# adeebkor/fenicsx-fus

Hardware: AMD Instinct MI355X
Metric: DOF-updates/sec (RK4 step) at p=4 hex fp64 (higher is better)
Workload: dtype f64; 1 GPU; 3D homogeneous wave, hex p=4 f64, Linear RK4, weak scaling: 64^3 cells per GPU (BASELINE.json configs[1]); ndofs_global=16974593, cells_per_gpu=262144, medium=water, partition=x-slabs x1, transport=none, blocks=8192, mfma_contractions=False, mfma_4x4x4_index1=False, packed_fp32=False, lds_bytes_per_block=72504

## Files before the change

fenicsx-fus_amd/csrc/fusmi.hip:

```cpp
#include <dlfcn.h>

#include <algorithm>
#include <cmath>
#include <cstdio>
#include <cstring>
#include <limits>
#include <memory>

#include "core.hpp"
#include "tables.hpp"

using namespace fus;

FUS_HIDDEN thread_local std::string g_err;
#define NCCLCHK(expr)                                                                              \
  do                                                                                               \
  {                                                                                                \
    ncclResult_t r_ = (expr);                                                                      \
    if (r_ != ncclSuccess)                                                                         \
      return fail(FUS_ERR_RCCL, std::string(#expr) + ": " + g_rccl.GetErrorString(r_));            \
  } while (0)

struct RcclApi
{
// ... 177 lines not shown
  const int Nd = op->Nd, ng = op->tdim == 3 ? 6 : 3;
  FUSCHK(dalloc_bytes(op->allocs, &op->d_G, (size_t)op->ncells * ng * Nd * sizeof(T), false, st));
  FUSCHK(dalloc_bytes(op->allocs, &op->d_detJ, (size_t)op->ncells * Nd * sizeof(T), false, st));
  return degree_impl(op->dtype, op->P)->stream_geometry(op);
}

static OpFacts op_facts(const fus_op* op, int mode, bool ortho, int deterministic)
{
  const fus_ctx* c = op->ctx;
  return {op->P, (int)op->ts, op->tdim, op->geom_order, mode, ortho, deterministic != 0, c->mfma, c->pack32, c->diag_metric};
}

template <typename T>
static int op_setup_device(fus_op* op)
{
  if (!degree_impl(op->dtype, op->P))
    return fail(FUS_ERR_ARG, "unsupported polynomial degree (2..10)");
  const int N = op->N;
  fus_ctx* c = op->ctx;
  hipStream_t st = c->stream;
  Layout& L = op->L;
  auto& pool = op->allocs;

  std::vector<ShapeDev> shapes(L.shapes.size());
  for (size_t i = 0; i < shapes.size(); ++i)
  {
    shapes[i].nelem = L.shapes[i].nelem, shapes[i].nloc = L.shapes[i].nloc;
    shapes[i].nint = L.shapes[i].nint, shapes[i].nrounds = L.shapes[i].nrounds;
    shapes[i].rounds_off = L.shapes[i].rounds_off, shapes[i].ldm_off = L.shapes[i].ldm_off;
  }
  int32_t *d_blk_shape, *d_elem_off, *d_int_off, *d_sh_gidx;
  int64_t* d_sh_off;
  ShapeDev* d_shapes;
  int16_t* d_rounds;
  uint16_t* d_ldm;
  FUSCHK(upload(pool, &d_blk_shape, L.blk_shape, st));
  FUSCHK(upload(pool, &d_shapes, shapes, st));
  FUSCHK(upload(pool, &d_elem_off, L.blk_elem_off, st));
  FUSCHK(upload(pool, &d_int_off, L.blk_int_off, st));
  FUSCHK(upload(pool, &d_sh_off, L.blk_sh_off, st));
  FUSCHK(upload(pool, &d_sh_gidx, L.sh_gidx, st));
  FUSCHK(upload(pool, &d_rounds, L.rounds, st));
  L.ldm.resize((L.ldm.size() + 15) & ~(size_t)15);
  FUSCHK(upload(pool, &d_ldm, L.ldm, st));
  FUSCHK(upload(pool, &op->d_cell_perm, L.cell_perm, st));
  FUSCHK(upload(pool, &op->d_dof_perm, L.dof_perm, st));
  FUSCHK(upload(pool, &op->d_sh_ptr, L.sh_ptr, st));
  {
    std::vector<int64_t> pos(L.sh_pairs.size());
    for (size_t k = 0; k < pos.size(); ++k)
      pos[k] = L.pair_pos[L.sh_pairs[k]];
    FUSCHK(upload(pool, &op->d_sh_pairs, pos, st));
  }
  int32_t* d_sh_ppos;
  FUSCHK(upload(pool, &d_sh_ppos, L.pair_pos, st));
  op->A.sh_ppos = d_sh_ppos;
  op->A.blk_shape = d_blk_shape, op->A.shapes = d_shapes, op->A.blk_elem_off = d_elem_off;
  op->A.blk_int_off = d_int_off, op->A.blk_sh_off = d_sh_off, op->A.sh_gidx = d_sh_gidx;
  op->A.rounds = d_rounds, op->A.ldm = d_ldm, op->A.nblocks = L.nblocks;
  op->A.lds_nloc = (L.max_nloc + 1) & ~1;
  op->A.waves = L.waves;
  op->A.lds_nelem = (L.max_nelem + 7) & ~7;
  op->lds_bytes = L.lds_bytes(sizeof(T), op->nfields);
  if (op->lds_bytes > 160 * 1024)
    return fail(FUS_ERR_LIMIT, "block does not fit 160 KB of LDS; lower block_elems");

  std::vector<T> Dg(N * N + 2 * N);
  for (int i = 0; i < N * N; ++i)
    Dg[i] = (T)op->D[i];
  for (int i = 0; i < N; ++i)
    Dg[N * N + i] = (T)op->wts[i], Dg[N * N + N + i] = (T)op->nodes[i];
  T* d_Dg;
  FUSCHK(upload(pool, &d_Dg, Dg, st));
  op->d_Dg = d_Dg;

  T* d_xg;
  FUSCHK(dalloc(pool, &d_xg, (size_t)op->nnodes * 3));
  HIPCHK(hipMemcpyAsync(d_xg, op->h_geom_x.data(), (size_t)op->nnodes * 3 * sizeof(T),
                        hipMemcpyHostToDevice, st));
  double *d_pts, *d_wts;
  FUSCHK(upload(pool, &op->d_xdm, op->h_geom_dm, st));
// ... 591 lines not shown
    const StageScalars scn = i < 3 ? stage_scalars<T>(m, i + 1, t, dt)
                                   : stage_scalars<T>(m, 0, (double)((T)t + (T)dt), dt);
    B.enabled = 1, B.npairs = (int32_t)op->L.n_partial;
    B.srcw = static_cast<const T*>(m->d_bsrc) + m->nb_int;
    B.absw = static_cast<const T*>(m->d_babs) + m->nb_int;
    B.src2w = m->d_bsrc2 ? static_cast<const T*>(m->d_bsrc2) + m->nb_int : nullptr;
    B.gnext = (T)scn.gval, B.dgnext = (T)scn.dgval;
    B.partial = static_cast<T*>(op->d_partial);
    m->bnd_valid = true, m->bnd_tn = scn.tn;
    op->bnd_owner = m;
    if (m->src_mode == 2)
    {
      B.gnext = T(1), B.dgnext = T(1);
      const bool need_int = !(m->src_tn_int == scn.tn);
      if (need_int || !(m->src_tn_sh == scn.tn))
        FUSCHK(source_entries<T>(m, need_int ? 0 : m->nb_int, m->nb, scn.tn));
    }
  }
  const LeanRK<T> R{(T)sc.b0dt, (T)sc.pdt, T(1) / T(3)};
  const int kind = stage_kind(m, i);
  if (nloc > 0 && c->planes && (int)op->L.plane_cnt.size() <= (c->planes == 1 ? FUS_MAX_PLANES : c->planes))
  {
    ProfScope ps(c, "stage");
    const dim3 grid(nblk(nloc)), blk(256);
    PartialPlanes PL{};
    PL.bnd0 = (int32_t)op->L.n_partial;
    for (size_t j = 0; j < op->L.plane_cnt.size(); ++j)
      PL.cnt[j] = (int32_t)op->L.plane_cnt[j], PL.off[j] = (int32_t)op->L.plane_off[j];
    FUSCHK(with_kind<FUS_STAGE_KINDS>(kind, [&](auto K) -> int
    {
      hipLaunchKernelGGL((k_shared_stage_planes<T, decltype(K)::value>), grid, blk, 0, st, nloc, PL, m->d_bnd_mask, m->d_bnd_base,
                         partial, minv + off, vn + off, un + off, u0 + off, v0 + off, u_ + off, v_ + off, adt, bdt,
                         m0p, mn1p, B, R);
      return FUS_OK;
    }));
  }
  else if (nloc > 0)
  {
    ProfScope ps(c, "stage");
    const dim3 grid(nblk(nloc)), blk(256);
    FUSCHK(with_kind<FUS_STAGE_KINDS>(kind, [&](auto K) -> int
    {
      hipLaunchKernelGGL((k_shared_stage<T, decltype(K)::value>), grid, blk, 0, st, nloc, m->d_sh_ptr32, m->d_sh_pairs32, partial,
                         minv + off, vn + off, un + off, u0 + off, v0 + off, u_ + off, v_ + off, adt, bdt, m0p, mn1p, B,
                         R);
      return FUS_OK;
    }));
// ... 1754 lines not shown
```

fenicsx-fus_amd/csrc/kernels.hpp:

```cpp
#pragma once
#include <hip/hip_runtime.h>
#include <stdint.h>

#include "block_variant.hpp"
#include "geom.hpp"
#include "source_wave.hpp"

namespace fus
{

struct ShapeDev
{
  int32_t nelem, nloc, nint, nrounds;
  int64_t rounds_off, ldm_off;
};

struct BlockArgs
{
  const int32_t* blk_shape;
  const ShapeDev* shapes;
  const int32_t* blk_elem_off;
  const int32_t* blk_int_off;
  const int64_t* blk_sh_off;
  const int32_t* sh_gidx;
  const int32_t* sh_ppos;
  const int16_t* rounds;
  const uint16_t* ldm;
  int32_t nblocks;
  int32_t blk_begin;
  int32_t blk_count;
  int32_t lds_nloc;
  int32_t lds_nelem;
  int32_t waves;
};

template <typename T>
struct StageArgs
{
  const T* minv;
  T *vn, *un, *u0, *v0, *u_, *v_;
  T adt, bdt, gval;
  T b0dt, pdt, third;
  const int32_t* blk_bnd_off;
  const int32_t* bnd_idx;
  const T* bnd_src;
  const T* bnd_abs;
// ... 1854 lines not shown
    for (int j = 0; j < N; ++j)
      acc += Dcc[j] * sA[a * N2 + b * N + j];
    Y[a] = acc;
  }
#pragma unroll
  for (int a = 0; a < N; ++a)
  {
    if (ATOMIC)
      __hip_atomic_fetch_add(&y_l[li[a]], (double)Y[a], __ATOMIC_RELAXED, __HIP_MEMORY_SCOPE_WORKGROUP);
    else
      y_l[li[a]] += Y[a];
  }
}

#define FUS_PF1(T, P, OP, ATOMIC, GEOM, TD)                                                         \
  (((P) >= 5 && (P) <= 7 && (OP) == OP_STIFFNESS && (GEOM) == GEOM_STREAM && (TD) == 3) ? 1 : 0)

template <typename T>
struct LeanRK
{
  T b0dt, pdt, third;
};

template <typename T, int STAGE>
__device__ __forceinline__ T stage_update_dof(int64_t s, T acc, const T* __restrict__ minv,
                                                 T* __restrict__ vn, T* __restrict__ un,
                                                 T* __restrict__ u0, T* __restrict__ v0,
                                                 T* __restrict__ u_, T* __restrict__ v_, T adt, T bdt,
                                                 const T* __restrict__ m0, const T* __restrict__ mn1,
                                                 const LeanRK<T> R)
{
#define FUS_LD(p) __builtin_nontemporal_load(&(p)[s])
#define FUS_ST(p, val) __builtin_nontemporal_store((val), &(p)[s])
  T kv;
  if (mn1)
  {
    const T us = stage_is_first(STAGE) ? u0[s] : un[s], vs = stage_is_first(STAGE) ? v0[s] : vn[s];
    kv = (acc - mn1[s] * vs * vs) / (m0[s] + mn1[s] * us);
  }
  else
    kv = acc * FUS_LD(minv);
  T vnext;
  if (STAGE == 0)
  {
    const T u = FUS_LD(u0), v = FUS_LD(v0);
    FUS_ST(u_, v * bdt + u);
    FUS_ST(v_, kv * bdt + v);
    FUS_ST(un, v * adt + u);
    vnext = kv * adt + v;
    FUS_ST(vn, vnext);
  }
  else if (STAGE == 4)
  {
    const T u = FUS_LD(u0), v = FUS_LD(v0);
    FUS_ST(un, v * adt + u);
    vnext = kv * adt + v;
    FUS_ST(v_, vnext);
  }
  else if (STAGE == 3)
  {
    FUS_ST(u0, FUS_LD(vn) * bdt + FUS_LD(u_));
    vnext = kv * bdt + FUS_LD(v_);
    FUS_ST(v0, vnext);
  }
  else if (STAGE == 5)
  {
    const T w = FUS_LD(vn), v = FUS_LD(v0), xs = FUS_LD(un);
    FUS_ST(un, xs + (w * adt - v * R.pdt));
    vnext = kv * adt + v;
    FUS_ST(v_, vnext);
  }
  else if (STAGE == 6)
  {
    const T w = FUS_LD(vn), v = FUS_LD(v0), va = FUS_LD(u_), xs = FUS_LD(un);
    FUS_ST(un, xs + (w * adt - va * R.pdt));
    vnext = kv * adt + v;
    FUS_ST(v_, vnext);
  }
  else if (STAGE == 7)
  {
    const T w = FUS_LD(vn), v = FUS_LD(v0), va = FUS_LD(u_), vb = FUS_LD(v_), xs = FUS_LD(un);
    FUS_ST(u0, (xs - vb * R.pdt) + ((va + vb) * T(2) + (v + w)) * R.b0dt);
    vnext = kv * bdt + ((vb * T(2) + (va + w)) - v) * R.third;
    FUS_ST(v0, vnext);
  }
  else
  {
    const T w = FUS_LD(vn);
    FUS_ST(u_, w * bdt + FUS_LD(u_));
    FUS_ST(v_, kv * bdt + FUS_LD(v_));
    FUS_ST(un, w * adt + FUS_LD(u0));
    vnext = kv * adt + FUS_LD(v0);
    FUS_ST(vn, vnext);
  }
#undef FUS_LD
#undef FUS_ST
  return vnext;
}

template <typename T, int N>
struct KArgs
{
  BlockArgs A;
  DTab<T, N> Dk;
  const T* Dg;
  const T* geo;
  const T* coef;
  const T* x;
  T* bvec;
  T* partial;
  StageArgs<T> S;
};

template <typename T, int N>
__device__ __forceinline__ void load_stage_args(const KArgs<T, N> __attribute__((address_space(4))) * q, StageArgs<T>& S)
{
  S.minv = q->S.minv;
  S.vn = q->S.vn, S.un = q->S.un, S.u0 = q->S.u0, S.v0 = q->S.v0, S.u_ = q->S.u_, S.v_ = q->S.v_;
  S.adt = q->S.adt, S.bdt = q->S.bdt, S.gval = q->S.gval;
  S.b0dt = q->S.b0dt, S.pdt = q->S.pdt, S.third = q->S.third;
  S.blk_bnd_off = q->S.blk_bnd_off, S.bnd_idx = q->S.bnd_idx;
// ... 49 lines not shown
  uint16_t* ldm_l = reinterpret_cast<uint16_t*>(w_l + (GCS ? (N <= 8 ? 16 : 24) : 0));  \
  int16_t* rt_l = reinterpret_cast<int16_t*>(ldm_l + (size_t)lds_nelem * Nd);                      \
  (void)y_l, (void)x2_l, (void)scratch, (void)D_l, (void)cf_l, (void)cf2_l, (void)gc_l, (void)w_l, (void)pt_l,      \
      (void)ldm_l, (void)rt_l, (void)slots

  const int tid0 = threadIdx.x, nthr = blockDim.x;
#define FUS_TID()                                                                                  \
  int tid = tid0;                                                                                  \
  asm volatile("" : "+v"(tid))
#define FUS_LANE_COORDS(q)                                                                         \
  FUS_TID();                                                                                       \
  const int lane = tid % LPE, wave = tid / LPE;         \
  const int s = lane / N2, p = lane - s * N2;                                                      \
  const int b = p / N, c = p - b * N;                                                              \
  const bool active = s < EPW;                                                                     \
  const int myslot = (wave * EPW + (active ? s : 0)) * EPS;                                        \
                                \
  T* sA = reinterpret_cast<T*>(smem_raw) + (size_t)((NF == 2 ? 2 : 1) + AW) * q->A.lds_nloc         \
          + (size_t)myslot * SLOT;                                                                 \
  T* sB = sA

  struct Meta
  {
    ShapeDev sh;
    int elem_off, int_off;
    int64_t sh_off;
  };
  auto meta_of = [&](KP q, int bk) -> Meta
  {
    Meta M;
    M.sh = q->A.shapes[q->A.blk_shape[bk]];
    M.elem_off = q->A.blk_elem_off[bk];
    M.int_off = q->A.blk_int_off[bk];
    M.sh_off = q->A.blk_sh_off[bk];
    return M;
  };
  typedef T V2 __attribute__((ext_vector_type(2)));
  typedef uint32_t U4 __attribute__((ext_vector_type(4)));
  constexpr int UI = (P <= 3) ? 3 : ((P == 4) ? 2 : (P <= 6 ? 4 : (P == 7 ? FUS_UI_P7 : FUS_UI_HI))),
                US = (P <= 3) ? 4 : ((P == 4) ? 3 : (P <= 7 ? 5 : FUS_UI_HI)),
                UL = (P <= 3) ? 2 : ((P == 4) ? 1 : 4);
  struct PLoad
  {
    V2 xi[UI], xi2[UI];
    T xs[US], xs2[US];
    U4 lq[UL];
    T cfv, cf2v, gcv, gcv2, dgv, xtail, xtail2;
  };
  auto p_idx = [&](KP q, const Meta& M, bool enable, int (&gi)[US]) __attribute__((always_inline))
  {
    FUS_TID();
    const int nsh = M.sh.nloc - M.sh.nint;
    const int32_t* gix = q->A.sh_gidx + M.sh_off;
#pragma unroll
    for (int u = 0; u < US; ++u)
      gi[u] = (enable && tid + u * nthr < nsh) ? gix[tid + u * nthr] : -1;
  };
  auto p_load = [&](KP q, const Meta& M, PLoad& L, bool with_tables, bool enable, const int (&gi)[US])
      __attribute__((always_inline))
  {
    FUS_TID();
    const ShapeDev& sh = M.sh;
    const T* __restrict__ x = q->x;
    const T* __restrict__ x2 = (NF == 2) ? q->S.x2 : x;
    const T* __restrict__ coef = q->coef;
    const T* __restrict__ coef2 = (NF == 2) ? q->S.coef2 : coef;
    const T* __restrict__ geo = q->geo;
    const T* __restrict__ Dg = q->Dg;
    const V2* xg = reinterpret_cast<const V2*>(x + M.int_off);
    const V2* xg2 = reinterpret_cast<const V2*>(x2 + M.int_off);
    const int nvec = sh.nint >> 1;
    const int nsh = sh.nloc - sh.nint;
    const int32_t* gix = q->A.sh_gidx + M.sh_off;
    const int n16 = (sh.nelem * Nd * 2 + 15) >> 4;
    const U4* lsrc = reinterpret_cast<const U4*>(q->A.ldm + sh.ldm_off);
    const int ngc = sh.nelem * GCS;
#pragma unroll
    for (int u = 0; u < UI; ++u)
    {
      const bool ok = enable && tid + u * nthr < nvec;
      L.xi[u] = ok ? xg[tid + u * nthr] : V2(T(0));
      L.xi2[u] = (NF == 2 && ok) ? xg2[tid + u * nthr] : V2(T(0));
    }
#pragma unroll
    for (int u = 0; u < UL; ++u)
      L.lq[u] = (enable && tid + u * nthr < n16) ? lsrc[tid + u * nthr] : U4(0u);
    L.cfv = (enable && tid < sh.nelem) ? coef[M.elem_off + tid] : T(0);
    L.cf2v = (NF == 2 && enable && tid < sh.nelem) ? coef2[M.elem_off + tid] : T(0);
    L.gcv = (enable && tid < ngc) ? geo[(int64_t)M.elem_off * GCS + tid] : T(0);
    L.gcv2 = (GCS > 7 && enable && tid + nthr < ngc) ? geo[(int64_t)M.elem_off * GCS + tid + nthr] : T(0);
    L.dgv = (with_tables && enable && tid < N2 + 2 * N) ? Dg[tid] : T(0);
    L.xtail = (enable && tid == 0 && (sh.nint & 1)) ? x[M.int_off + sh.nint - 1] : T(0);
    L.xtail2 = (NF == 2 && enable && tid == 0 && (sh.nint & 1)) ? x2[M.int_off + sh.nint - 1] : T(0);
#pragma unroll
    for (int u = 0; u < US; ++u)
    {
      L.xs[u] = gi[u] >= 0 ? x[gi[u]] : T(0);
      L.xs2[u] = (NF == 2 && gi[u] >= 0) ? x2[gi[u]] : T(0);
    }
  };
  auto p_commit = [&](KP q, const Meta& M, const PLoad& L, bool with_tables) __attribute__((always_inline))
  {
    FUS_PHASE_LDS(q);
    FUS_TID();
    const ShapeDev& sh = M.sh;
    const T* __restrict__ x = q->x;
    const T* __restrict__ x2 = (NF == 2) ? q->S.x2 : x;
    const T* __restrict__ coef = q->coef;
    const T* __restrict__ coef2 = (NF == 2) ? q->S.coef2 : coef;
    const T* __restrict__ geo = q->geo;
    const T* __restrict__ Dg = q->Dg;
    const V2* xg = reinterpret_cast<const V2*>(x + M.int_off);
    const V2* xg2 = reinterpret_cast<const V2*>(x2 + M.int_off);
    const int nvec = sh.nint >> 1;
    const int nsh = sh.nloc - sh.nint;
    const int32_t* gix = q->A.sh_gidx + M.sh_off;
    const int n16 = (sh.nelem * Nd * 2 + 15) >> 4;
    const U4* lsrc = reinterpret_cast<const U4*>(q->A.ldm + sh.ldm_off);
    const int ngc = sh.nelem * GCS;
    for (int i = tid; i < (sh.nloc + 1) / 2; i += nthr)
      reinterpret_cast<A2*>(y_l)[i] = A2(0.0);
#pragma unroll
    for (int u = 0; u < UI; ++u)
      if (tid + u * nthr < nvec)
      {
        reinterpret_cast<V2*>(x_l)[tid + u * nthr] = L.xi[u];
        if (NF == 2)
          reinterpret_cast<V2*>(x2_l)[tid + u * nthr] = L.xi2[u];
// ... 111 lines not shown
      gc_l[k] = geo[(int64_t)M.elem_off * GCS + k];
    if (!ATOMIC)
      for (int k = tid; k < sh.nrounds * slots; k += nthr)
        rt_l[k] = q->A.rounds[sh.rounds_off + k];
  };

  FUS_KARGS(q0);
  const int blk_end = q0->A.blk_begin + q0->A.blk_count;
  const int blk_stride = gridDim.x;
  int wg = blockIdx.x;
  if (FUS_XCD_REMAP)
  {
    const int G = gridDim.x, q8 = G >> 3, r8 = G & 7, xc = wg & 7;
    wg = xc * q8 + (xc < r8 ? xc : r8) + (wg >> 3);
  }
  int blk = wg + q0->A.blk_begin;
  FUS_STAMP(blk, 0);
  ElemIn<T, N, OP, GEOM, TD> inA, inB;
  auto first_fetch = [&](KP q, const Meta& Mm) __attribute__((always_inline))
  {
    FUS_LANE_COORDS(q);
    (void)b, (void)c, (void)sA, (void)sB;
    const int slots = (q->A.waves * 64 / LPE) * EPW * EPS;
    const int nt0 = ATOMIC ? (Mm.sh.nelem + slots - 1) / slots : Mm.sh.nrounds;
    int e0 = -1;
    if (active && nt0 > 0)
      e0 = ATOMIC ? (myslot < Mm.sh.nelem ? myslot : -1) : (int)q->A.rounds[Mm.sh.rounds_off + myslot];
    elem_fetch<T, N, OP, GEOM, TD>(inA, e0, q->geo, Mm.elem_off, p);
  };
  PLoad L;
  {
    const Meta M0 = meta_of(q0, blk);
    first_fetch(q0, M0);
    int gi0[US];
    p_idx(q0, M0, true, gi0);
    p_load(q0, M0, L, true, true, gi0);
  }
  bool first = true;
  for (;;)
  {
  FUS_KARGS(qc);
  FUS_PHASE_LDS(qc);
  FUS_LANE_COORDS(qc);
  const Meta M = meta_of(qc, blk);
  const ShapeDev& sh = M.sh;
  const int elem_off = M.elem_off;
  const int ntrips = ATOMIC ? (sh.nelem + slots - 1) / slots : sh.nrounds;
  auto elem_of = [&](int r) -> int
  {
    if (!active || r >= ntrips)
      return -1;
    if (ATOMIC)
      return (r * slots + myslot < sh.nelem) ? r * slots + myslot : -1;
    return (int)rt_l[r * slots + myslot];
  };
#ifdef FUS_PROBE_PFREE
  if (first)
    p_commit(qc, M, L, true);
  else
  {
    FUS_TID();
    for (int i = tid; i < (M.sh.nloc + 1) / 2; i += nthr)
      reinterpret_cast<A2*>(y_l)[i] = A2(0.0);
  }
#else
  p_commit(qc, M, L, first);
#endif
  const int blk_next = blk + blk_stride;
  const bool has_next = blk_next < blk_end;
  constexpr bool IDX_EARLY = false;
  int gi_n[US];
  if constexpr (IDX_EARLY)
  {
    Meta Mi{};
    if (has_next)
      Mi = meta_of(qc, blk_next);
    p_idx(qc, Mi, has_next, gi_n);
  }
  __syncthreads();
  FUS_STAMP(blk, 1);
#ifdef FUS_STAGGER
  if (tid0 >= 256)
    __builtin_amdgcn_s_sleep(FUS_STAGGER);
#endif
  T Drb[N], Drc[N], Dcb[N], Dcc[N], w3[N];
// ... 83 lines not shown
    FUS_ELEM_COMPUTE(inA);
    if (r == 0)
      FUS_STAMP(blk, 5);
    if (r == 2)
      FUS_STAMP(blk, 7);
    if (!ATOMIC && nwaves > 1)
      __syncthreads();
    elem_fetch<T, N, OP, GEOM, TD>(inA, elem_of(r + 2), geo, elem_off, p);
    if (has1)
    {
      FUS_ELEM_COMPUTE(inB);
      if (r == 0)
        FUS_STAMP(blk, 6);
      if (!ATOMIC && nwaves > 1)
        __syncthreads();
    }
  }
#undef FUS_ELEM_COMPUTE
  {
  FUS_KARGS(qe);
  FUS_PHASE_LDS(qe);
  FUS_TID();
  const Meta M = meta_of(qe, blk);
  const ShapeDev& sh = M.sh;
  const int int_off = M.int_off;
  const int64_t sh_off = M.sh_off;
  StageArgs<T> S;
  load_stage_args<T, N>(qe, S);
  T* __restrict__ bvec = qe->bvec;
  T* __restrict__ partial = qe->partial;
  const int32_t* __restrict__ pp = qe->A.sh_ppos + sh_off;
  const int nsh = sh.nloc - sh.nint;
  int ppv[US];
#pragma unroll
  for (int u = 0; u < US; ++u)
    ppv[u] = (tid + u * nthr < nsh) ? pp[tid + u * nthr] : -1;

  const int nvec = sh.nint >> 1;
    constexpr bool EPI2 = (P <= 4) && (NF == 1);
    struct Epi
    {
      bool on;
      int i, o;
      V2 bv, mi, w, a0, b0, au, av, m1, m0v, us;
    };
    auto epi_load = [&](int i, Epi& E, int part) __attribute__((always_inline))
    {
      if (part != 2)
      {
      E.on = i < nvec;
      E.i = i, E.o = int_off + 2 * i;
      E.bv = E.mi = E.w = E.a0 = E.b0 = E.au = E.av = E.m1 = E.m0v = E.us = V2(T(0));
#ifdef FUS_PROBE_EFREE
      auto ld = [&](const T* ptr) -> V2 { return E.on ? V2(T(1)) + V2(T((uintptr_t)ptr & 7)) : V2(T(0)); };
#else
      auto ld = [&](const T* ptr) -> V2
      { return E.on ? __builtin_nontemporal_load(reinterpret_cast<const V2*>(ptr + E.o)) : V2(T(0)); };
#endif
      constexpr bool WV = NF == 2;
// ... 100 lines not shown
#ifdef FUS_PROBE_PFREE
    if constexpr (!IDX_EARLY)
      p_idx(qn, Mn, false, gi_n);
    p_load(qn, Mn, L, false, false, gi_n);
#else
    if constexpr (!IDX_EARLY)
      p_idx(qn, Mn, has_next, gi_n);
    p_load(qn, Mn, L, false, has_next, gi_n);
#endif
  }
  if (STAGE == STAGE_NONE)
  {
    V2* bg = reinterpret_cast<V2*>(bvec + int_off);
    for (int i = tid; i < nvec; i += nthr)
    {
      const A2 a2 = reinterpret_cast<const A2*>(y_l)[i];
      bg[i] = V2{(T)a2[0], (T)a2[1]};
    }
    if (tid == 0 && (sh.nint & 1))
      bvec[int_off + sh.nint - 1] = (T)y_l[sh.nint - 1];
  }
  else
  {
    const int k0 = S.blk_bnd_off[blk], k1 = S.blk_bnd_off[blk + 1];
    if (k1 > k0)
    {
      const T* vstage = stage_is_first(STAGE) ? S.v0 : S.vn;
      for (int k = k0 + tid; k < k1; k += nthr)
      {
        const int gi = S.bnd_idx[k];
        T add = S.gval * S.bnd_src[k] - S.bnd_abs[k] * vstage[gi];
        if (NF == 2)
          add += S.dgval * S.bnd_src2[k];
        y_l[gi - int_off] += add;
      }
      __syncthreads();
    }
    if (tid == 0 && (sh.nint & 1))
      (void)stage_update_dof<T, STAGE>((int64_t)int_off + sh.nint - 1, (T)y_l[sh.nint - 1], S.minv, S.vn, S.un, S.u0,
                                       S.v0, S.u_, S.v_, S.adt, S.bdt, (NF == 2) ? S.m0 : nullptr,
                                       (NF == 2) ? S.mn1 : nullptr, LeanRK<T>{S.b0dt, S.pdt, S.third});
#pragma unroll
    for (int u = 0; u < EPIU; ++u)
      epi_load(tid + u * nthr, Ef[u], EARLY ? 2 : 0);
#pragma unroll
    for (int u = 0; u < EPIU; ++u)
      epi_store(Ef[u]);
// ... 41 lines not shown
{
  const int64_t s = s0 + (int64_t)blockIdx.x * blockDim.x + threadIdx.x;
  if (s >= s1)
    return;
  T acc = T(0);
  for (I k = sh_ptr[s]; k < sh_ptr[s + 1]; ++k)
    acc += partial[sh_pairs[k]];
  bsh[s] = acc;
}

template <typename T>
struct BndNext
{
  int enabled;
  int32_t npairs;
  const T *srcw, *absw, *src2w;
  T gnext, dgnext;
  T* partial;
};

template <typename T>
__device__ __forceinline__ void boundary_next(const BndNext<T>& B, int32_t last_pair, T vnext)
{
  if (B.enabled && last_pair >= B.npairs)
  {
    const int32_t k = last_pair - B.npairs;
    T v = B.gnext * B.srcw[k] - B.absw[k] * vnext;
    if (B.src2w)
      v += B.dgnext * B.src2w[k];
    B.partial[last_pair] = v;
  }
}



constexpr int FUS_MAX_PLANES = 16;
struct PartialPlanes
{
  int32_t bnd0;
  int32_t cnt[FUS_MAX_PLANES];
  int32_t off[FUS_MAX_PLANES];
};

template <typename T, int STAGE>
__global__ void __launch_bounds__(256)
k_shared_stage_planes(int64_t n, const PartialPlanes PL, const uint64_t* __restrict__ bnd_mask,
                      const int32_t* __restrict__ bnd_base, const T* __restrict__ partial,
                      const T* __restrict__ minv, T* __restrict__ vn, T* __restrict__ un, T* __restrict__ u0,
                      T* __restrict__ v0, T* __restrict__ u_, T* __restrict__ v_, T adt, T bdt,
                      const T* __restrict__ m0, const T* __restrict__ mn1, const BndNext<T> B, const LeanRK<T> R)
{
  const int64_t s = (int64_t)blockIdx.x * blockDim.x + threadIdx.x;
  if (s >= n)
    return;
  T acc = T(0);
#pragma unroll
  for (int j = 0; j < FUS_MAX_PLANES; ++j)
  {
    if (s < PL.cnt[j])
      acc += partial[(int64_t)PL.off[j] + s];
  }
  int32_t pair = -1;
  if (bnd_mask)
  {
    const uint64_t w = bnd_mask[s >> 6];
    const int bit = (int)(s & 63);
    if ((w >> bit) & 1ull)
    {
      pair = PL.bnd0 + bnd_base[s >> 6] + __builtin_popcountll(w & ((1ull << bit) - 1ull));
      acc += partial[pair];
    }
  }
  const T vnext = stage_update_dof<T, STAGE>(s, acc, minv, vn, un, u0, v0, u_, v_, adt, bdt, m0, mn1, R);
  boundary_next<T>(B, pair, vnext);
}

template <typename T, int STAGE>
__global__ void __launch_bounds__(256)
k_shared_stage(int64_t n, const int32_t* __restrict__ sh_ptr, const int32_t* __restrict__ sh_pairs,
               const T* __restrict__ partial, const T* __restrict__ minv, T* __restrict__ vn,
               T* __restrict__ un, T* __restrict__ u0, T* __restrict__ v0, T* __restrict__ u_,
               T* __restrict__ v_, T adt, T bdt, const T* __restrict__ m0,
               const T* __restrict__ mn1, const BndNext<T> B, const LeanRK<T> R)
{
  const int64_t s = (int64_t)blockIdx.x * blockDim.x + threadIdx.x;
  if (s >= n)
    return;
  T acc = T(0);
  int32_t pair = 0;
  for (int32_t k = sh_ptr[s]; k < sh_ptr[s + 1]; ++k)
  {
    pair = sh_pairs[k];
    acc += partial[pair];
  }
  const T vnext = stage_update_dof<T, STAGE>(s, acc, minv, vn, un, u0, v0, u_, v_, adt, bdt, m0, mn1, R);
  boundary_next<T>(B, pair, vnext);
}
// ... 428 lines not shown
```

fenicsx-fus_amd/csrc/layout.cpp:

```cpp
#include "layout.hpp"

#include <algorithm>
#include <cstring>
#include <map>
#include <numeric>
#include <unordered_map>

namespace fus
{
namespace
{
struct Rcb
{
  const double* cen;
  std::vector<int32_t>& order;
  std::vector<std::pair<int64_t, int64_t>>& leaves;

  void split(int64_t lo, int64_t hi, int64_t nparts)
  {
    if (nparts <= 1 || hi - lo <= 1)
    {
      leaves.emplace_back(lo, hi);
      return;
    }
// ... 328 lines not shown
        const int64_t mid = (lo + hi) / 2;
        if (L.sh_ptr[mid + 1] - L.sh_ptr[mid] > j)
          lo = mid + 1;
        else
          hi = mid;
      }
      cnt = lo;
    }
    if (cnt == 0)
      break;
    L.plane_cnt.push_back(cnt), L.plane_off.push_back(cursor);
    cursor = (cursor + cnt + 15) & ~(int64_t)15;
  }
  L.pair_pos.assign(L.npairs, -1);
  for (int64_t sidx = 0; sidx < L.n_shared_local; ++sidx)
    for (int64_t k = L.sh_ptr[sidx]; k < L.sh_ptr[sidx + 1]; ++k)
      L.pair_pos[L.sh_pairs[k]] = (int32_t)(L.plane_off[k - L.sh_ptr[sidx]] + sidx);
  const int64_t if_first = L.sh_ptr[std::min(L.n_if_start_pad, L.n_shared)];
  for (int64_t k = if_first; k < L.npairs; ++k)
    L.pair_pos[L.sh_pairs[k]] = (int32_t)(cursor + (k - if_first));
  L.n_partial = cursor + (L.npairs - if_first);
  if (L.n_partial + L.n_shared > 2000000000ll)
    return "partial slab exceeds int32 indexing";
  return "";
}

std::string verify_layout(const Layout& L, const int32_t* dm)
{
  const int Nd = L.Nd;
  {
    std::vector<uint8_t> seen(L.ncells, 0);
    for (int64_t e = 0; e < L.ncells; ++e)
    {
      const int32_t c = L.cell_perm[e];
      if (c < 0 || c >= L.ncells || seen[c])
        return "cell_perm is not a permutation";
      seen[c] = 1;
    }
  }
  {
    std::vector<uint8_t> seen(L.n_internal, 0);
    for (int64_t g = 0; g < L.ndofs; ++g)
    {
      const int32_t p = L.dof_perm[g];
      if (p < 0 || p >= L.n_internal || seen[p])
        return "dof_perm is not injective";
      seen[p] = 1;
// ... 34 lines not shown
        if (e >= sh.nelem || used[e]++)
          return "round table does not cover each element once";
        for (int i = 0; i < Nd; ++i)
          if (stamp[L.ldm[sh.ldm_off + (int64_t)e * Nd + i]] == r)
            return "two elements of one round share a dof";
        for (int i = 0; i < Nd; ++i)
          stamp[L.ldm[sh.ldm_off + (int64_t)e * Nd + i]] = r;
      }
    for (int e = 0; e < sh.nelem; ++e)
      if (!used[e])
        return "element missing from rounds";
    pairs_seen += sh.nloc - sh.nint;
  }
  if (pairs_seen != L.npairs)
    return "pair count mismatch";
  {
    std::vector<char> taken(L.n_partial, 0);
    for (int64_t k = 0; k < L.npairs; ++k)
    {
      if (L.pair_pos[k] < 0 || L.pair_pos[k] >= L.n_partial || taken[L.pair_pos[k]]++)
        return "two pairs share a partial position";
    }
  }
  for (int64_t s = 0; s < L.n_shared; ++s)
    for (int64_t k = L.sh_ptr[s]; k < L.sh_ptr[s + 1]; ++k)
    {
      if (L.sh_gidx[L.sh_pairs[k]] != L.n_int_pad + s)
        return "shared CSR inconsistent";
      if (k > L.sh_ptr[s] && L.sh_pairs[k] <= L.sh_pairs[k - 1])
        return "shared CSR not in ascending block order";
      const int64_t pos = L.pair_pos[L.sh_pairs[k]], j = k - L.sh_ptr[s];
      if (pos < 0 || pos >= L.n_partial)
        return "partial position out of range";
      if (s < L.n_shared_local && (j >= (int64_t)L.plane_cnt.size() || s >= L.plane_cnt[j] || pos != L.plane_off[j] + s))
        return "partial position is not (plane of the sharer's rank, dof index)";
    }
  return "";
}

}
```

fenicsx-fus_amd/csrc/layout.hpp:

```cpp
#pragma once
#include <cstdint>
#include <string>
#include <vector>

namespace fus
{

struct Layout
{
  int P = 0, N = 0, Nd = 0;
  int tdim = 3;
  int waves = 4;
  int epw = 1;
  int slots = 4;
  int64_t ncells = 0, ndofs = 0;

  int32_t nblocks = 0;
  int32_t nblocks_if = 0;
  std::vector<int32_t> cell_perm;
  std::vector<int32_t> blk_elem_off;

  struct Shape
  {
    int32_t nelem, nloc, nint, nrounds;
    int64_t rounds_off;
    int64_t ldm_off;
  };
  std::vector<Shape> shapes;
  std::vector<int32_t> blk_shape;
  std::vector<int16_t> rounds;
  std::vector<uint16_t> ldm;

  std::vector<int32_t> dof_perm;
  std::vector<int32_t> blk_int_off;
  std::vector<int64_t> blk_sh_off;
  std::vector<int32_t> sh_gidx;
  int64_t n_int_pad = 0;
  int64_t n_interior = 0, n_shared = 0, npairs = 0;
  int64_t n_shared_local = 0, n_if_start_pad = 0;
  int64_t n_internal = 0;
  std::vector<int64_t> sh_ptr;
  std::vector<int64_t> sh_pairs;
  std::vector<int32_t> pair_pos;
  std::vector<int64_t> plane_cnt, plane_off;
  int64_t n_partial = 0;
  int32_t max_nloc = 0, max_rounds = 0, max_nelem = 0;

  size_t lds_bytes(size_t sizeofT, int nfields = 1, int geom_cell_stride = 0) const
  {
    const size_t ne = ((size_t)max_nelem + 7) & ~(size_t)7;
    return (size_t)nfields * ((max_nloc + 1) & ~1) * sizeofT
           + (size_t)((max_nloc + 1) & ~1) * 8
           + (size_t)slots * ((tdim == 3 && N == 7 && sizeofT == 4) ? N * 56 : Nd + N) * sizeofT
           + (size_t)N * N * sizeofT + nfields * ne * sizeofT
           + (geom_cell_stride ? ((size_t)geom_cell_stride * ne + (N <= 8 ? 16 : 24)) * sizeofT : 0)
           + ne * Nd * 2
           + (size_t)max_rounds * slots * 2 + 16;
  }
};

std::string build_layout(Layout& L, int P, int64_t ncells, int64_t ndofs,
                         const int32_t* tensor_dofmap, const double* centroids, int block_elems,
                         int waves, const uint8_t* force_shared = nullptr, int tdim = 3, int slot_factor = 1);

std::string verify_layout(const Layout& L, const int32_t* tensor_dofmap);

}
```

Baseline: 13.71 billion DOF-updates/s.

## Vectorize shared-DOF stage update and pack per-block metadata into cache-line records

The shared/plane stage kernel now handles several DOFs per thread (16-byte vectors) and uses vector nontemporal loads and stores for partial planes and the RK state arrays, with scalar fallbacks for tails. Per-block metadata that used to be gathered from five separate arrays is packed into one 64-byte BlockRecord and read through the constant address space. The boundary offsets are also loaded early, and the RK update arithmetic is rewritten with explicit FMAs under fp contract(off). In return the code adds a plane-alignment requirement and changes rounding slightly because of the explicit FMAs.

```diff
diff --git a/fenicsx-fus_amd/csrc/fusmi.hip b/fenicsx-fus_amd/csrc/fusmi.hip
--- a/fenicsx-fus_amd/csrc/fusmi.hip
+++ b/fenicsx-fus_amd/csrc/fusmi.hip
@@ -223,23 +223,11 @@
   Layout& L = op->L;
   auto& pool = op->allocs;
 
-  std::vector<ShapeDev> shapes(L.shapes.size());
-  for (size_t i = 0; i < shapes.size(); ++i)
-  {
-    shapes[i].nelem = L.shapes[i].nelem, shapes[i].nloc = L.shapes[i].nloc;
-    shapes[i].nint = L.shapes[i].nint, shapes[i].nrounds = L.shapes[i].nrounds;
-    shapes[i].rounds_off = L.shapes[i].rounds_off, shapes[i].ldm_off = L.shapes[i].ldm_off;
-  }
-  int32_t *d_blk_shape, *d_elem_off, *d_int_off, *d_sh_gidx;
-  int64_t* d_sh_off;
-  ShapeDev* d_shapes;
+  int32_t* d_sh_gidx;
+  BlockRecord* d_blk_rec;
   int16_t* d_rounds;
   uint16_t* d_ldm;
-  FUSCHK(upload(pool, &d_blk_shape, L.blk_shape, st));
-  FUSCHK(upload(pool, &d_shapes, shapes, st));
-  FUSCHK(upload(pool, &d_elem_off, L.blk_elem_off, st));
-  FUSCHK(upload(pool, &d_int_off, L.blk_int_off, st));
-  FUSCHK(upload(pool, &d_sh_off, L.blk_sh_off, st));
+  FUSCHK(upload(pool, &d_blk_rec, L.blk_rec, st));
   FUSCHK(upload(pool, &d_sh_gidx, L.sh_gidx, st));
   FUSCHK(upload(pool, &d_rounds, L.rounds, st));
   L.ldm.resize((L.ldm.size() + 15) & ~(size_t)15);
@@ -256,8 +244,7 @@
   int32_t* d_sh_ppos;
   FUSCHK(upload(pool, &d_sh_ppos, L.pair_pos, st));
   op->A.sh_ppos = d_sh_ppos;
-  op->A.blk_shape = d_blk_shape, op->A.shapes = d_shapes, op->A.blk_elem_off = d_elem_off;
-  op->A.blk_int_off = d_int_off, op->A.blk_sh_off = d_sh_off, op->A.sh_gidx = d_sh_gidx;
+  op->A.blk_rec = d_blk_rec, op->A.sh_gidx = d_sh_gidx;
   op->A.rounds = d_rounds, op->A.ldm = d_ldm, op->A.nblocks = L.nblocks;
   op->A.lds_nloc = (L.max_nloc + 1) & ~1;
   op->A.waves = L.waves;
@@ -895,7 +882,8 @@
   if (nloc > 0 && c->planes && (int)op->L.plane_cnt.size() <= (c->planes == 1 ? FUS_MAX_PLANES : c->planes))
   {
     ProfScope ps(c, "stage");
-    const dim3 grid(nblk(nloc)), blk(256);
+    constexpr int W = 16 / (int)sizeof(T);
+    const dim3 grid(nblk((nloc + W - 1) / W)), blk(256);
     PartialPlanes PL{};
     PL.bnd0 = (int32_t)op->L.n_partial;
     for (size_t j = 0; j < op->L.plane_cnt.size(); ++j)
diff --git a/fenicsx-fus_amd/csrc/kernels.hpp b/fenicsx-fus_amd/csrc/kernels.hpp
--- a/fenicsx-fus_amd/csrc/kernels.hpp
+++ b/fenicsx-fus_amd/csrc/kernels.hpp
@@ -4,24 +4,15 @@
 
 #include "block_variant.hpp"
 #include "geom.hpp"
+#include "layout.hpp"
 #include "source_wave.hpp"
 
 namespace fus
 {
 
-struct ShapeDev
-{
-  int32_t nelem, nloc, nint, nrounds;
-  int64_t rounds_off, ldm_off;
-};
-
 struct BlockArgs
 {
-  const int32_t* blk_shape;
-  const ShapeDev* shapes;
-  const int32_t* blk_elem_off;
-  const int32_t* blk_int_off;
-  const int64_t* blk_sh_off;
+  const BlockRecord* blk_rec;
   const int32_t* sh_gidx;
   const int32_t* sh_ppos;
   const int16_t* rounds;
@@ -1922,81 +1913,181 @@
   T b0dt, pdt, third;
 };
 
+enum : int { SR_MINV = 1, SR_M0 = 2, SR_MN1 = 4, SR_U0 = 8, SR_V0 = 16, SR_UN = 32, SR_VN = 64, SR_UA = 128, SR_VA = 256 };
+__host__ __device__ constexpr int stage_reads(int st, bool wv)
+{
+  return ((st == 0 || st == 4) ? SR_U0 | SR_V0
+          : st == 3            ? SR_VN | SR_UA | SR_VA
+          : st == 5            ? SR_VN | SR_V0 | SR_UN
+          : st == 6            ? SR_VN | SR_V0 | SR_UA | SR_UN
+          : st == 7            ? SR_VN | SR_V0 | SR_UA | SR_VA | SR_UN
+                               : SR_VN | SR_UA | SR_VA | SR_U0 | SR_V0)
+         | (wv ? SR_M0 | SR_MN1 | (stage_is_first(st) ? SR_U0 | SR_V0 : SR_UN | SR_VN) : SR_MINV);
+}
+__host__ __device__ constexpr int stage_writes(int st)
+{
+  return (st == 3 || st == 7) ? SR_U0 | SR_V0 : (st >= 4 ? SR_UN | SR_VA : SR_UA | SR_VA | SR_UN | SR_VN);
+}
+
+template <typename T>
+struct StageRegs
+{
+  T minv, m0, mn1, u0, v0, un, vn, ua, va;
+};
+
+__device__ __forceinline__ double fmadd(double a, double b, double c) { return __builtin_fma(a, b, c); }
+__device__ __forceinline__ float fmadd(float a, float b, float c) { return __builtin_fmaf(a, b, c); }
+
+__host__ __device__ constexpr int stage_kv_reads(int st, bool wv)
+{
+  return wv ? SR_M0 | SR_MN1 | (stage_is_first(st) ? SR_U0 | SR_V0 : SR_UN | SR_VN) : SR_MINV;
+}
 template <typename T, int STAGE>
-__device__ __forceinline__ T stage_update_dof(int64_t s, T acc, const T* __restrict__ minv,
+__device__ __forceinline__ T stage_kv(T acc, bool wv, const StageRegs<T>& r)
+{
+#pragma clang fp contract(off)
+  if (wv)
+  {
+    const T us = stage_is_first(STAGE) ? r.u0 : r.un, vs = stage_is_first(STAGE) ? r.v0 : r.vn;
+    return fmadd(-vs, r.mn1 * vs, acc) / fmadd(r.mn1, us, r.m0);
+  }
+  return acc * r.minv;
+}
+template <typename T, int STAGE>
+__device__ __forceinline__ T stage_finish(T kv, StageRegs<T>& r, T adt, T bdt, const LeanRK<T> R)
+{
+#pragma clang fp contract(off)
+  T vnext;
+  if (STAGE == 0)
+  {
+    const T u = r.u0, v = r.v0;
+    r.ua = fmadd(v, bdt, u);
+    r.va = fmadd(kv, bdt, v);
+    r.un = fmadd(v, adt, u);
+    vnext = fmadd(kv, adt, v);
+    r.vn = vnext;
+  }
+  else if (STAGE == 4)
+  {
+    const T u = r.u0, v = r.v0;
+    r.un = fmadd(v, adt, u);
+    vnext = fmadd(kv, adt, v);
+    r.va = vnext;
+  }
+  else if (STAGE == 3)
+  {
+    r.u0 = fmadd(r.vn, bdt, r.ua);
+    vnext = fmadd(kv, bdt, r.va);
+    r.v0 = vnext;
+  }
+  else if (STAGE == 5)
+  {
+    const T w = r.vn, v = r.v0, xs = r.un;
+    r.un = xs + fmadd(w, adt, -(v * R.pdt));
+    vnext = fmadd(kv, adt, v);
+    r.va = vnext;
+  }
+  else if (STAGE == 6)
+  {
+    const T w = r.vn, v = r.v0, va = r.ua, xs = r.un;
+    r.un = xs + fmadd(w, adt, -(va * R.pdt));
+    vnext = fmadd(kv, adt, v);
+    r.va = vnext;
+  }
+  else if (STAGE == 7)
+  {
+    const T w = r.vn, v = r.v0, va = r.ua, vb = r.va, xs = r.un;
+    r.u0 = fmadd(fmadd(va + vb, T(2), v + w), R.b0dt, fmadd(-vb, R.pdt, xs));
+    vnext = fmadd(kv, bdt, (fmadd(vb, T(2), va + w) - v) * R.third);
+    r.v0 = vnext;
+  }
+  else
+  {
+    const T w = r.vn, ua = r.ua, va = r.va;
+    r.ua = fmadd(w, bdt, ua);
+    r.va = fmadd(kv, bdt, va);
+    r.un = fmadd(w, adt, r.u0);
+    vnext = fmadd(kv, adt, r.v0);
+    r.vn = vnext;
+  }
+  return vnext;
+}
+template <typename T, int STAGE>
+__device__ __forceinline__ T stage_update_regs(T acc, bool wv, StageRegs<T>& r, T adt, T bdt, const LeanRK<T> R)
+{
+  return stage_finish<T, STAGE>(stage_kv<T, STAGE>(acc, wv, r), r, adt, bdt, R);
+}
+
+#define FUS_STAGE_VECTORS(X)                                                                        \
+  X(minv, minv, SR_MINV) X(m0, m0, SR_M0) X(mn1, mn1, SR_MN1) X(u0, u0, SR_U0) X(v0, v0, SR_V0)     \
+  X(un, un, SR_UN) X(vn, vn, SR_VN) X(ua, u_, SR_UA) X(va, v_, SR_VA)
+template <typename T, int STAGE, typename V = T>
+__device__ __forceinline__ V stage_update_dof(int64_t s, V acc, const T* __restrict__ minv,
                                                  T* __restrict__ vn, T* __restrict__ un,
                                                  T* __restrict__ u0, T* __restrict__ v0,
                                                  T* __restrict__ u_, T* __restrict__ v_, T adt, T bdt,
                                                  const T* __restrict__ m0, const T* __restrict__ mn1,
-                                                 const LeanRK<T> R)
-{
-#define FUS_LD(p) __builtin_nontemporal_load(&(p)[s])
-#define FUS_ST(p, val) __builtin_nontemporal_store((val), &(p)[s])
-  T kv;
-  if (mn1)
-  {
-    const T us = stage_is_first(STAGE) ? u0[s] : un[s], vs = stage_is_first(STAGE) ? v0[s] : vn[s];
-    kv = (acc - mn1[s] * vs * vs) / (m0[s] + mn1[s] * us);
+                                                 const LeanRK<T> R, int nv = (int)(sizeof(V) / sizeof(T)))
+{
+  constexpr int W = (int)(sizeof(V) / sizeof(T));
+  const bool wv = mn1 != nullptr;
+  const bool whole = W == 1 || nv == W;
+  StageRegs<V> q{};
+  const int reads = stage_reads(STAGE, wv);
+  auto load = [&](int mask) __attribute__((always_inline))
+  {
+#define FUS_LD(f, p, bit)                                                                           \
+  if (reads & mask & (bit))                                                                         \
+  {                                                                                                 \
+    if (whole)                                                                                      \
+      q.f = __builtin_nontemporal_load(reinterpret_cast<const V*>(&(p)[s]));                        \
+    else if constexpr (W > 1)                                                                       \
+      for (int e = 0; e < W; ++e)                                                                   \
+        if (e < nv)                                                                                 \
+          q.f[e] = __builtin_nontemporal_load(&(p)[s + e]);                                         \
+  }
+    FUS_STAGE_VECTORS(FUS_LD)
+#undef FUS_LD
+  };
+  V vnext;
+  if constexpr (W == 1)
+  {
+    load(stage_kv_reads(STAGE, wv));
+    const T kv = stage_kv<T, STAGE>(acc, wv, q);
+    load(~stage_kv_reads(STAGE, wv));
+    vnext = stage_finish<T, STAGE>(kv, q, adt, bdt, R);
   }
   else
-    kv = acc * FUS_LD(minv);
-  T vnext;
-  if (STAGE == 0)
-  {
-    const T u = FUS_LD(u0), v = FUS_LD(v0);
-    FUS_ST(u_, v * bdt + u);
-    FUS_ST(v_, kv * bdt + v);
-    FUS_ST(un, v * adt + u);
-    vnext = kv * adt + v;
-    FUS_ST(vn, vnext);
-  }
-  else if (STAGE == 4)
-  {
-    const T u = FUS_LD(u0), v = FUS_LD(v0);
-    FUS_ST(un, v * adt + u);
-    vnext = kv * adt + v;
-    FUS_ST(v_, vnext);
-  }
-  else if (STAGE == 3)
-  {
-    FUS_ST(u0, FUS_LD(vn) * bdt + FUS_LD(u_));
-    vnext = kv * bdt + FUS_LD(v_);
-    FUS_ST(v0, vnext);
-  }
-  else if (STAGE == 5)
-  {
-    const T w = FUS_LD(vn), v = FUS_LD(v0), xs = FUS_LD(un);
-    FUS_ST(un, xs + (w * adt - v * R.pdt));
-    vnext = kv * adt + v;
-    FUS_ST(v_, vnext);
-  }
-  else if (STAGE == 6)
-  {
-    const T w = FUS_LD(vn), v = FUS_LD(v0), va = FUS_LD(u_), xs = FUS_LD(un);
-    FUS_ST(un, xs + (w * adt - va * R.pdt));
-    vnext = kv * adt + v;
-    FUS_ST(v_, vnext);
-  }
-  else if (STAGE == 7)
-  {
-    const T w = FUS_LD(vn), v = FUS_LD(v0), va = FUS_LD(u_), vb = FUS_LD(v_), xs = FUS_LD(un);
-    FUS_ST(u0, (xs - vb * R.pdt) + ((va + vb) * T(2) + (v + w)) * R.b0dt);
-    vnext = kv * bdt + ((vb * T(2) + (va + w)) - v) * R.third;
-    FUS_ST(v0, vnext);
-  }
-  else
-  {
-    const T w = FUS_LD(vn);
-    FUS_ST(u_, w * bdt + FUS_LD(u_));
-    FUS_ST(v_, kv * bdt + FUS_LD(v_));
-    FUS_ST(un, w * adt + FUS_LD(u0));
-    vnext = kv * adt + FUS_LD(v0);
-    FUS_ST(vn, vnext);
-  }
-#undef FUS_LD
+  {
+    load(~0);
+#pragma unroll
+    for (int e = 0; e < W; ++e)
+    {
+      StageRegs<T> r;
+#define FUS_GET(f, p, bit) r.f = q.f[e];
+      FUS_STAGE_VECTORS(FUS_GET)
+#undef FUS_GET
+      vnext[e] = stage_update_regs<T, STAGE>(acc[e], wv, r, adt, bdt, R);
+#define FUS_PUT(f, p, bit) q.f[e] = r.f;
+      FUS_STAGE_VECTORS(FUS_PUT)
+#undef FUS_PUT
+    }
+  }
+#define FUS_ST(f, p, bit)                                                                           \
+  if constexpr ((stage_writes(STAGE) & (bit)) != 0)                                                 \
+  {                                                                                                 \
+    if (whole)                                                                                      \
+      __builtin_nontemporal_store(q.f, reinterpret_cast<V*>(const_cast<T*>(&(p)[s])));              \
+    else if constexpr (W > 1)                                                                       \
+      for (int e = 0; e < W; ++e)                                                                   \
+        if (e < nv)                                                                                 \
+          __builtin_nontemporal_store(q.f[e], const_cast<T*>(&(p)[s + e]));                         \
+  }
+  FUS_STAGE_VECTORS(FUS_ST)
 #undef FUS_ST
   return vnext;
 }
+#undef FUS_STAGE_VECTORS
 
 template <typename T, int N>
 struct KArgs
@@ -2092,17 +2183,19 @@
 
   struct Meta
   {
-    ShapeDev sh;
-    int elem_off, int_off;
+    int32_t elem_off, int_off;
     int64_t sh_off;
+    int32_t nelem, nloc, nint, nrounds;
+    int64_t rounds_off, ldm_off;
   };
   auto meta_of = [&](KP q, int bk) -> Meta
   {
+    const BlockRecord __attribute__((address_space(4)))* r
+        = (const BlockRecord __attribute__((address_space(4)))*)q->A.blk_rec + bk;
     Meta M;
-    M.sh = q->A.shapes[q->A.blk_shape[bk]];
-    M.elem_off = q->A.blk_elem_off[bk];
-    M.int_off = q->A.blk_int_off[bk];
-    M.sh_off = q->A.blk_sh_off[bk];
+    M.elem_off = r->elem_off, M.int_off = r->int_off, M.sh_off = r->sh_off;
+    M.nelem = r->nelem, M.nloc = r->nloc, M.nint = r->nint, M.nrounds = r->nrounds;
+    M.rounds_off = r->rounds_off, M.ldm_off = r->ldm_off;
     return M;
   };
   typedef T V2 __attribute__((ext_vector_type(2)));
@@ -2120,7 +2213,7 @@
   auto p_idx = [&](KP q, const Meta& M, bool enable, int (&gi)[US]) __attribute__((always_inline))
   {
     FUS_TID();
-    const int nsh = M.sh.nloc - M.sh.nint;
+    const int nsh = M.nloc - M.nint;
     const int32_t* gix = q->A.sh_gidx + M.sh_off;
 #pragma unroll
     for (int u = 0; u < US; ++u)
@@ -2130,7 +2223,7 @@
       __attribute__((always_inline))
   {
     FUS_TID();
-    const ShapeDev& sh = M.sh;
+    const Meta& sh = M;
     const T* __restrict__ x = q->x;
     const T* __restrict__ x2 = (NF == 2) ? q->S.x2 : x;
     const T* __restrict__ coef = q->coef;
@@ -2173,7 +2266,7 @@
   {
     FUS_PHASE_LDS(q);
     FUS_TID();
-    const ShapeDev& sh = M.sh;
+    const Meta& sh = M;
     const T* __restrict__ x = q->x;
     const T* __restrict__ x2 = (NF == 2) ? q->S.x2 : x;
     const T* __restrict__ coef = q->coef;
@@ -2331,10 +2424,10 @@
     FUS_LANE_COORDS(q);
     (void)b, (void)c, (void)sA, (void)sB;
     const int slots = (q->A.waves * 64 / LPE) * EPW * EPS;
-    const int nt0 = ATOMIC ? (Mm.sh.nelem + slots - 1) / slots : Mm.sh.nrounds;
+    const int nt0 = ATOMIC ? (Mm.nelem + slots - 1) / slots : Mm.nrounds;
     int e0 = -1;
     if (active && nt0 > 0)
-      e0 = ATOMIC ? (myslot < Mm.sh.nelem ? myslot : -1) : (int)q->A.rounds[Mm.sh.rounds_off + myslot];
+      e0 = ATOMIC ? (myslot < Mm.nelem ? myslot : -1) : (int)q->A.rounds[Mm.rounds_off + myslot];
     elem_fetch<T, N, OP, GEOM, TD>(inA, e0, q->geo, Mm.elem_off, p);
   };
   PLoad L;
@@ -2352,7 +2445,7 @@
   FUS_PHASE_LDS(qc);
   FUS_LANE_COORDS(qc);
   const Meta M = meta_of(qc, blk);
-  const ShapeDev& sh = M.sh;
+  const Meta& sh = M;
   const int elem_off = M.elem_off;
   const int ntrips = ATOMIC ? (sh.nelem + slots - 1) / slots : sh.nrounds;
   auto elem_of = [&](int r) -> int
@@ -2369,7 +2462,7 @@
   else
   {
     FUS_TID();
-    for (int i = tid; i < (M.sh.nloc + 1) / 2; i += nthr)
+    for (int i = tid; i < (M.nloc + 1) / 2; i += nthr)
       reinterpret_cast<A2*>(y_l)[i] = A2(0.0);
   }
 #else
@@ -2499,7 +2592,7 @@
   FUS_PHASE_LDS(qe);
   FUS_TID();
   const Meta M = meta_of(qe, blk);
-  const ShapeDev& sh = M.sh;
+  const Meta& sh = M;
   const int int_off = M.int_off;
   const int64_t sh_off = M.sh_off;
   StageArgs<T> S;
@@ -2512,6 +2605,12 @@
 #pragma unroll
   for (int u = 0; u < US; ++u)
     ppv[u] = (tid + u * nthr < nsh) ? pp[tid + u * nthr] : -1;
+  int bnd_k0 = 0, bnd_k1 = 0;
+  if (STAGE != STAGE_NONE)
+  {
+    const int32_t __attribute__((address_space(4)))* bo = (const int32_t __attribute__((address_space(4)))*)S.blk_bnd_off + blk;
+    bnd_k0 = bo[0], bnd_k1 = bo[1];
+  }
 
   const int nvec = sh.nint >> 1;
     constexpr bool EPI2 = (P <= 4) && (NF == 1);
@@ -2658,7 +2757,12 @@
   }
   else
   {
+#ifdef FUS_PROBE_BND_LATE
     const int k0 = S.blk_bnd_off[blk], k1 = S.blk_bnd_off[blk + 1];
+    (void)bnd_k0, (void)bnd_k1;
+#else
+    const int k0 = bnd_k0, k1 = bnd_k1;
+#endif
     if (k1 > k0)
     {
       const T* vstage = stage_is_first(STAGE) ? S.v0 : S.vn;
@@ -2746,12 +2850,13 @@
 template <typename T>
 __device__ __forceinline__ void boundary_next(const BndNext<T>& B, int32_t last_pair, T vnext)
 {
+#pragma clang fp contract(off)
   if (B.enabled && last_pair >= B.npairs)
   {
     const int32_t k = last_pair - B.npairs;
-    T v = B.gnext * B.srcw[k] - B.absw[k] * vnext;
+    T v = fmadd(B.gnext, B.srcw[k], -(B.absw[k] * vnext));
     if (B.src2w)
-      v += B.dgnext * B.src2w[k];
+      v = fmadd(B.dgnext, B.src2w[k], v);
     B.partial[last_pair] = v;
   }
 }
@@ -2774,29 +2879,64 @@
                       T* __restrict__ v0, T* __restrict__ u_, T* __restrict__ v_, T adt, T bdt,
                       const T* __restrict__ m0, const T* __restrict__ mn1, const BndNext<T> B, const LeanRK<T> R)
 {
-  const int64_t s = (int64_t)blockIdx.x * blockDim.x + threadIdx.x;
+  constexpr int W = 16 / (int)sizeof(T);
+  typedef T V __attribute__((ext_vector_type(W)));
+  const int64_t s = ((int64_t)blockIdx.x * blockDim.x + threadIdx.x) * W;
   if (s >= n)
     return;
-  T acc = T(0);
+  T acc[W];
+#pragma unroll
+  for (int e = 0; e < W; ++e)
+    acc[e] = T(0);
 #pragma unroll
   for (int j = 0; j < FUS_MAX_PLANES; ++j)
   {
-    if (s < PL.cnt[j])
-      acc += partial[(int64_t)PL.off[j] + s];
-  }
-  int32_t pair = -1;
+    const int64_t cnt = PL.cnt[j], off = PL.off[j];
+    if (s + W <= cnt)
+    {
+      const V v = __builtin_nontemporal_load(reinterpret_cast<const V*>(partial + off + s));
+#pragma unroll
+      for (int e = 0; e < W; ++e)
+        acc[e] += v[e];
+    }
+    else
+    {
+#pragma unroll
+      for (int e = 0; e < W; ++e)
+        if (s + e < cnt)
+          acc[e] += partial[off + s + e];
+    }
+  }
+  int32_t pair[W];
+#pragma unroll
+  for (int e = 0; e < W; ++e)
+    pair[e] = -1;
   if (bnd_mask)
   {
     const uint64_t w = bnd_mask[s >> 6];
-    const int bit = (int)(s & 63);
-    if ((w >> bit) & 1ull)
-    {
-      pair = PL.bnd0 + bnd_base[s >> 6] + __builtin_popcountll(w & ((1ull << bit) - 1ull));
-      acc += partial[pair];
-    }
-  }
-  const T vnext = stage_update_dof<T, STAGE>(s, acc, minv, vn, un, u0, v0, u_, v_, adt, bdt, m0, mn1, R);
-  boundary_next<T>(B, pair, vnext);
+    const int bit0 = (int)(s & 63);
+    if ((w >> bit0) & ((1ull << W) - 1ull))
+    {
+      const int32_t base = PL.bnd0 + bnd_base[s >> 6];
+#pragma unroll
+      for (int e = 0; e < W; ++e)
+        if ((w >> (bit0 + e)) & 1ull)
+        {
+          pair[e] = base + __builtin_popcountll(w & ((1ull << (bit0 + e)) - 1ull));
+          acc[e] += partial[pair[e]];
+        }
+    }
+  }
+  V av;
+#pragma unroll
+  for (int e = 0; e < W; ++e)
+    av[e] = acc[e];
+  const int nv = (n - s < W) ? (int)(n - s) : W;
+  const V vnext = stage_update_dof<T, STAGE, V>(s, av, minv, vn, un, u0, v0, u_, v_, adt, bdt, m0, mn1, R, nv);
+#pragma unroll
+  for (int e = 0; e < W; ++e)
+    if (e < nv)
+      boundary_next<T>(B, pair[e], vnext[e]);
 }
 
 template <typename T, int STAGE>
diff --git a/fenicsx-fus_amd/csrc/layout.cpp b/fenicsx-fus_amd/csrc/layout.cpp
--- a/fenicsx-fus_amd/csrc/layout.cpp
+++ b/fenicsx-fus_amd/csrc/layout.cpp
@@ -374,7 +374,22 @@
   L.n_partial = cursor + (L.npairs - if_first);
   if (L.n_partial + L.n_shared > 2000000000ll)
     return "partial slab exceeds int32 indexing";
+  L.blk_rec = block_records(L);
   return "";
+}
+
+std::vector<BlockRecord> block_records(const Layout& L)
+{
+  std::vector<BlockRecord> rec(L.nblocks);
+  for (int32_t b = 0; b < L.nblocks; ++b)
+  {
+    const Layout::Shape& sh = L.shapes[L.blk_shape[b]];
+    BlockRecord& r = rec[b];
+    r.elem_off = L.blk_elem_off[b], r.int_off = L.blk_int_off[b], r.sh_off = L.blk_sh_off[b];
+    r.nelem = sh.nelem, r.nloc = sh.nloc, r.nint = sh.nint, r.nrounds = sh.nrounds;
+    r.rounds_off = sh.rounds_off, r.ldm_off = sh.ldm_off;
+  }
+  return rec;
 }
 
 std::string verify_layout(const Layout& L, const int32_t* dm)
@@ -455,6 +470,11 @@
         return "two pairs share a partial position";
     }
   }
+  for (int64_t off : L.plane_off)
+    if (off % 16)
+      return "plane not aligned";
+  if ((int64_t)L.blk_rec.size() != L.nblocks)
+    return "block records missing";
   for (int64_t s = 0; s < L.n_shared; ++s)
     for (int64_t k = L.sh_ptr[s]; k < L.sh_ptr[s + 1]; ++k)
     {
diff --git a/fenicsx-fus_amd/csrc/layout.hpp b/fenicsx-fus_amd/csrc/layout.hpp
--- a/fenicsx-fus_amd/csrc/layout.hpp
+++ b/fenicsx-fus_amd/csrc/layout.hpp
@@ -5,6 +5,16 @@
 
 namespace fus
 {
+
+struct alignas(64) BlockRecord
+{
+  int32_t elem_off, int_off;
+  int64_t sh_off;
+  int32_t nelem, nloc, nint, nrounds;
+  int64_t rounds_off, ldm_off;
+  uint8_t pad[16] = {};
+};
+static_assert(sizeof(BlockRecord) == 64 && alignof(BlockRecord) == 64, "one cache line per block");
 
 struct Layout
 {
@@ -28,6 +38,7 @@
   };
   std::vector<Shape> shapes;
   std::vector<int32_t> blk_shape;
+  std::vector<BlockRecord> blk_rec;
   std::vector<int16_t> rounds;
   std::vector<uint16_t> ldm;
 
@@ -63,6 +74,8 @@
                          const int32_t* tensor_dofmap, const double* centroids, int block_elems,
                          int waves, const uint8_t* force_shared = nullptr, int tdim = 3, int slot_factor = 1);
 
+std::vector<BlockRecord> block_records(const Layout& L);
+
 std::string verify_layout(const Layout& L, const int32_t* tensor_dofmap);
 
 }
```

Result: faster. 15.21 billion DOF-updates/s, median of 6 (+10.9%).
